# aerius-labs/paillier-halo2

Measured on AMD Instinct MI355X. Metric: Paillier-encrypt proofs/s (2048-bit n, k=17); MSM achieved HBM GB/s vs peak, higher is better.
Workload: dtype u32 limbs (29-bit reduced radix, 254-bit modular integers), u64 limbs (4096-bit integers)

## Files before the change

### paillier_halo2_amd/csrc/pz_msm.hip

```cpp
#include "ec.cuh"
#include "ec29.cuh"
#include "ec29_quad.cuh"
#include <math.h>
#include <stdlib.h>

#include "pz_internal.h"

#define MSM_CHUNK_MIN 16u
#define MSM_CHUNK_MAX 256u
#define MSM_HEAVY 24u
#define MSM_MEDIUM 1024u
#define MSM_SLICE_MAX_COLS 8u

struct MsmP {
    size_t n;
    size_t n_table;
    unsigned c;
    unsigned nwin;
    unsigned win_lo, win_hi;
    unsigned B;
    size_t cap;
    size_t max_items;
    unsigned chunk;
    unsigned spt;
// ... 132 lines not shown
            for (unsigned w = 0; w < p.win_hi; ++w) {
                int d = next_digit(s, w, p.c, carry);
                if (w >= p.win_lo && d != 0) atomicAdd(&h[(d < 0 ? -d : d) - 1], 1u);
            }
        }
    }
    __syncthreads();
    u32* out = slice_hist + (col * n_slices + slice) * (size_t)p.B;
    for (unsigned b = threadIdx.x; b < p.B; b += SORT_THREADS) out[b] = h[b];
}

__global__ __launch_bounds__(256) void k_msm_totals(u32* __restrict__ slice_hist, unsigned n_slices, MsmP p,
                                                    u32* __restrict__ totals) {
    const size_t col = blockIdx.y;
    const unsigned b = blockIdx.x * blockDim.x + threadIdx.x;
    if (b >= p.B) return;
    u32* sh = slice_hist + col * n_slices * (size_t)p.B + b;
    u32 run = 0;
    unsigned sl = 0;
    for (; sl + 8 <= n_slices; sl += 8) {
        u32 v[8];
#pragma unroll
        for (unsigned k = 0; k < 8; ++k) v[k] = sh[(size_t)(sl + k) * p.B];
#pragma unroll
        for (unsigned k = 0; k < 8; ++k) {
            sh[(size_t)(sl + k) * p.B] = run;
            run += v[k];
        }
    }
    for (; sl < n_slices; ++sl) {
        const u32 v = sh[(size_t)sl * p.B];
        sh[(size_t)sl * p.B] = run;
        run += v;
    }
    totals[col * p.B + b] = run;
}

#define ITEMS_SOLO 64u
#define SCAN_THREADS 1024
__global__ __launch_bounds__(SCAN_THREADS) void k_msm_scan(const u32* __restrict__ hist, MsmP p, u32* __restrict__ offs,
                                                  u32* __restrict__ items, u32* __restrict__ heavy,
                                                  u32* __restrict__ heavy_cnt, u32* __restrict__ fold_order,
                                                  u32* __restrict__ fold_cnt, u32* __restrict__ item_order,
                                                  u32* __restrict__ item_bucket, unsigned long long* __restrict__ digits_total) {
    __shared__ u32 s_cnt[SCAN_THREADS], s_itm[SCAN_THREADS];
    __shared__ u32 s_heavy;
    __shared__ u32 s_bin[MSM_HEAVY + 1], s_base[MSM_HEAVY + 1];
    __shared__ u32 s_obin[MSM_CHUNK_MAX + 1], s_obase[MSM_CHUNK_MAX + 1];
    if (threadIdx.x == 0) s_heavy = 0;
    if (threadIdx.x <= MSM_HEAVY) s_bin[threadIdx.x] = 0;
    for (unsigned t = threadIdx.x; t <= MSM_CHUNK_MAX; t += blockDim.x) s_obin[t] = 0;
    __syncthreads();
    const size_t col = blockIdx.x;
    const u32* h = hist + col * p.B;
    u32* o = offs + col * (p.B + 1);
    u32* it = items + col * (p.B + 1);
    const unsigned per = (p.B + SCAN_THREADS - 1) / SCAN_THREADS;
    const unsigned lo = threadIdx.x * per;
    u32 hv[32];
#pragma unroll
    for (unsigned k = 0; k < 32; ++k) hv[k] = (k < per && lo + k < p.B) ? h[lo + k] : 0u;
    u32 c = 0, m = 0;
#pragma unroll
    for (unsigned k = 0; k < 32; ++k) {
        const unsigned b = lo + k;
        if (k < per && b < p.B) {
// ... 62 lines not shown
            it[b] = m;
            c += v;
            const u32 ch = (v + p.chunk - 1) / p.chunk;
            m += ch;
            if (ch > 1 && ch <= MSM_HEAVY) fold_order[col * p.B + s_base[ch] + atomicAdd(&s_bin[ch], 1u)] = b;
            if (ch) {
                const u32 q = v / ch, rem = v % ch;
                const u32 ph = rem ? s_obase[q + 1] + atomicAdd(&s_obin[q + 1], rem) : 0u;
                const u32 pl = s_obase[q] + atomicAdd(&s_obin[q], ch - rem);
                {
                    const u32 item0 = m - ch;
                    u32* ord = item_order + col * p.max_items;
                    u32* obk = item_bucket + col * p.max_items;
                    for (u32 j = 0; j < ch; ++j) {
                        const u32 pos = j < rem ? ph + j : pl + j - rem;
                        ord[pos] = item0 + j;
                        obk[pos] = b;
                    }
                }
            }
        }
    }
}

#define SORT_FINE_LOG 7u
#define SORT_FINE (1u << SORT_FINE_LOG)
#define SORT_COARSE_MAX (SORT_MAXB >> SORT_FINE_LOG)
#define COARSE_THREADS 256u
#define COARSE_ROUND (COARSE_THREADS * 16u)
static_assert(COARSE_ROUND <= 65536u && SORT_COARSE_MAX <= 256u && SORT_COARSE_MAX == COARSE_THREADS, "k_msm_scatter_coarse packing");
__global__ __launch_bounds__(COARSE_THREADS) void k_msm_scatter_coarse(const Fr* __restrict__ scalars, size_t col_stride, MsmP p,
                                                                       const u32* __restrict__ slice_hist, unsigned n_slices,
                                                                       const u32* __restrict__ offs, u32* __restrict__ staged,
                                                                       size_t n_cols, ScatterSel sel) {
    if (!scatter_dense(sel)) return;
    __shared__ u32 cb[SORT_COARSE_MAX];
    __shared__ u32 cnt[SORT_COARSE_MAX];
    __shared__ u32 lbase[SORT_COARSE_MAX];
    __shared__ u32 gb[SORT_COARSE_MAX];
    __shared__ u32 stage[COARSE_ROUND];
    __shared__ unsigned char sbin[COARSE_ROUND];
    __shared__ u32 s_total;
    size_t col;
    unsigned slice;
    if (!sort_block_coords(n_slices, n_cols, slice, col)) return;
    const u32* in = slice_hist + (col * n_slices + slice) * (size_t)p.B;
    const u32* o = offs + col * (p.B + 1);
    const unsigned n_coarse = p.B >> SORT_FINE_LOG;
    if (threadIdx.x < SORT_COARSE_MAX) {
        cb[threadIdx.x] = threadIdx.x < n_coarse ? o[threadIdx.x << SORT_FINE_LOG] : 0u;
        cnt[threadIdx.x] = 0;
    }
    __syncthreads();
    for (unsigned b0 = (threadIdx.x & ~63u); b0 < p.B; b0 += 4 * COARSE_THREADS) {
        u32 v[4];
#pragma unroll
        for (unsigned k = 0; k < 4; ++k) {
            const unsigned b = b0 + k * COARSE_THREADS + (threadIdx.x & 63u);
            v[k] = b < p.B ? in[b] : 0u;
        }
#pragma unroll
        for (unsigned k = 0; k < 4; ++k) {
            u32 t = v[k];
#pragma unroll
            for (int off = 32; off > 0; off >>= 1) t += __shfl_xor(t, off, 64);
            const unsigned b = b0 + k * COARSE_THREADS;
            if ((threadIdx.x & 63u) == 0 && b < p.B && t) atomicAdd(&cb[b >> SORT_FINE_LOG], t);
        }
    }
    __syncthreads();
    u32* e = staged + col * p.cap;
    const size_t base = (size_t)slice * SORT_THREADS * p.spt;
    const unsigned rounds = SORT_THREADS * p.spt / COARSE_THREADS;
    Fr nxt = fp_zero<FrTag>();
    if (base + threadIdx.x < p.n) nxt = fp_load<FrTag>(scalars + col * col_stride + base + threadIdx.x);
    for (unsigned rd = 0; rd < rounds; ++rd) {
        const size_t i = base + (size_t)rd * COARSE_THREADS + threadIdx.x;
        if (base + (size_t)rd * COARSE_THREADS >= p.n) break;
        const Fr cur_scalar = nxt;
        u32 ev[16], rb[16];
#pragma unroll
        for (unsigned w = 0; w < 16; ++w) rb[w] = 0xffffffffu;
        if (i < p.n) {
            u32 s[8];
            const bool neg = scalar_prepare(cur_scalar, s);
            unsigned carry = 0;
#pragma unroll
// ... 719 lines not shown
    size_t i = (size_t)blockIdx.x * blockDim.x + threadIdx.x;
    if (i >= n) return;
    G1A29 a = x29_to_affine(x29_load_jac(in + i));
    if (!a29_is_inf(a)) {
        a.x = f29_to_256(a.x);
        a.y = f29_to_256(a.y);
    }
    a29_store64(out + i, a);
}

__global__ __launch_bounds__(128) void k_fixed_base_mul(const Fr* __restrict__ scalars, size_t n,
                                                        G1Aff64* __restrict__ out) {
    size_t i = (size_t)blockIdx.x * blockDim.x + threadIdx.x;
    if (i >= n) return;
    Fr k = fp_from_mont(fp_load<FrTag>(scalars + i));
    G1A29 g;
    g.x = f29_one<FqTag>();
    g.y = f29_canon<1>(f29_dbl(g.x));
    G1X29 acc = x29_inf();
    for (int bit = 253; bit >= 0; --bit) {
        acc = x29_dbl(acc);
        u32 w = sel8(k.v, (unsigned)bit >> 5);
        if ((w >> (bit & 31)) & 1) x29_add_affine(acc, g);
    }
    G1A29 a = x29_to_affine(acc);
    if (!a29_is_inf(a)) {
        a.x = f29_to_256(a.x);
        a.y = f29_to_256(a.y);
    }
    a29_store64(out + i, a);
}

static size_t pz_msm_ws_gib() {
    static size_t v = 0;
    if (!v) {
        const char* e = getenv("PZ_MSM_WS_GIB");
        long g = e ? atol(e) : 48;
        v = g < 1 ? 1 : (size_t)g;
    }
    return v;
}

static unsigned default_window_bits(size_t n) {
    if (n <= 1u << 8) return 9;
    if (n <= 1u << 11) return 11;
    if (n <= 1u << 14) return 13;
    return 16;
}

extern "C" int pz_bases_load_g1(pz_ctx* ctx, const uint64_t* bases_affine, size_t n_points, int on_device,
                                uint32_t window_bits, pz_bases** out) {
    if (!ctx || !out || !bases_affine || n_points == 0) return PZ_ERR_INVALID;
    *out = nullptr;
    unsigned c = window_bits ? window_bits : default_window_bits(n_points);
    if (c < 4 || c > 16) return PZ_ERR_INVALID;
    unsigned nwin = 253 / c + 1;
    if ((uint64_t)nwin * n_points >= (1ull << 31)) return PZ_ERR_UNSUPPORTED;
    PZ_ENTER(ctx);
    pz_bases* b = new pz_bases();
    b->n = n_points;
    b->c = c;
    b->nwin = nwin;
    b->device = ctx->device;
    hipError_t e = pz_hip_malloc(ctx, &b->d_table, (size_t)nwin * n_points * 64);
    if (e != hipSuccess) {
        delete b;
        return pz_hip_fail(ctx, e, "hipMalloc(table)");
    }
    const void* d_src = bases_affine;
    if (!on_device) {
        void* stage;
        int rc = pz_ws_get(ctx, WS_IO_A, n_points * 64, &stage);
        if (rc != PZ_OK) { (void)pz_hip_free(b->d_table); delete b; return rc; }
// ... 50 lines not shown
        unsigned c32 = ch < 24.0 ? MSM_CHUNK_MIN : 32u * (unsigned)((ch + 16.0) / 32.0);
        if (c32 > MSM_CHUNK_MAX) c32 = MSM_CHUNK_MAX;
        return c32;
    }
    const size_t want = (n_cols * digits_per_col) >> 18;
    unsigned chunk = MSM_CHUNK_MIN;
    while (chunk < MSM_CHUNK_MAX && chunk * 2 <= want) chunk *= 2;
    return chunk;
}

static unsigned msm_spt_for(size_t n_cols, size_t n) {
    const size_t min_wg = n_cols <= MSM_SLICE_MAX_COLS ? 128 : 512;
    unsigned spt = SORT_PER_THREAD;
    while (spt > 1 && n_cols * pz_div_up(n, (size_t)SORT_THREADS * spt) < min_wg) spt >>= 1;
    return spt;
}

#ifndef MSM_SPARSE_SLICE
#define MSM_SPARSE_SLICE (1u << 15)
#endif
static unsigned msm_spt_sparse(size_t n_cols, size_t n) {
    static long env = -1;
    if (env < 0) {
        const char* e = getenv("PZ_MSM_SPARSE_SLICE");
        env = e ? atol(e) : 0;
    }
    const size_t slice = env >= (long)SORT_SLICE && env <= (1l << 24) ? (size_t)env : (size_t)MSM_SPARSE_SLICE;
    unsigned spt = SORT_PER_THREAD;
    while ((size_t)SORT_THREADS * spt * 2 <= slice && (size_t)SORT_THREADS * spt < n) spt <<= 1;
    while (spt > 1 && n_cols * pz_div_up(n, (size_t)SORT_THREADS * spt) < 512) spt >>= 1;
    return spt;
}

static int msm_group(pz_ctx* ctx, const pz_bases* bases, const Fr* d_scalars, size_t nc, size_t n, size_t cs,
                     unsigned win_lo, unsigned win_hi, unsigned chunk, int density, G1Jac* d_out) {
    MsmP p;
    p.n = n;
    p.n_table = bases->n;
    p.c = bases->c;
    p.nwin = bases->nwin;
    p.win_lo = win_lo;
    p.win_hi = win_hi;
    p.B = 1u << (bases->c - 1);
    p.cap = n * (size_t)(win_hi - win_lo);
    p.chunk = chunk;
    if (p.B + n * (size_t)(win_hi - win_lo) / chunk > 65535u * 256u) return PZ_ERR_CAPACITY;
    p.max_items = p.B + p.cap / chunk;
    void *hist, *offs, *heavy, *items, *entries, *partials, *na, *nb, *totals, *fold, *iord;
    static int scatter_mode = -1;
    if (scatter_mode < 0) {
        const char* e = getenv("PZ_MSM_SCATTER");
        scatter_mode = (e && !strcmp(e, "one")) ? 1 : (e && !strcmp(e, "two")) ? 2 : 0;
    }
    const bool batch = nc > MSM_SLICE_MAX_COLS;
    const bool hint_sparse = batch && scatter_mode == 0 && density == PZ_MSM_SPARSE;
    const bool hint_dense = batch && scatter_mode == 0 && density == PZ_MSM_DENSE;
    p.spt = hint_sparse ? msm_spt_sparse(nc, n) : msm_spt_for(nc, n);
    const unsigned n_slices = pz_div_up(n, (size_t)SORT_THREADS * p.spt);
    const bool one_slice = hint_sparse && n_slices == 1;
    PZCHK(pz_ws_get(ctx, WS_HIST, nc * (size_t)n_slices * p.B * 4, &hist));
    PZCHK(pz_ws_get(ctx, WS_CURSOR, nc * (size_t)(p.B + 1) * 4, &heavy));
    const bool split_items = nc <= MSM_SLICE_MAX_COLS;
    const unsigned nblk_few = pz_div_up(p.B, 256);
    PZCHK(pz_ws_get(ctx, WS_TOTALS, nc * ((size_t)p.B + (split_items ? (size_t)nblk_few * (2 + FEW_BINS) : 0)) * 4, &totals));
    u32* blk_cnt = (u32*)totals + nc * (size_t)p.B;
    u32* blk_itm = blk_cnt + nc * (size_t)nblk_few;
    u32* blk_bins = blk_itm + nc * (size_t)nblk_few;
    u32* heavy_cnt = (u32*)heavy + nc * (size_t)p.B;
    PZCHK(pz_ws_get(ctx, WS_MISC, nc * (size_t)(p.B + 1) * 4, &fold));
    u32* fold_cnt = (u32*)fold + nc * (size_t)p.B;
    PZCHK(pz_ws_get(ctx, WS_ORDER, nc * p.max_items * 8, &iord));
    u32* item_order = (u32*)iord;
    u32* item_bucket = (u32*)iord + nc * p.max_items;
    PZCHK(pz_ws_get(ctx, WS_OFFS, nc * (p.B + 1) * 4, &offs));
    PZCHK(pz_ws_get(ctx, WS_ITEMS, nc * (p.B + 1) * 4, &items));
    PZCHK(pz_ws_get(ctx, WS_ENTRIES, nc * p.cap * 4 + 16, &entries));
    const bool two_pass = scatter_mode != 1 && !hint_sparse && p.c == 16 && (size_t)p.nwin * p.n_table <= ((size_t)1 << 24) &&
                          (nc > MSM_SLICE_MAX_COLS || scatter_mode == 2);
    {
        const size_t part_bytes = nc * p.max_items * sizeof(G1X29Raw), stage_bytes = two_pass ? nc * p.cap * 4 + 16 : 0;
        PZCHK(pz_ws_get(ctx, WS_PARTIALS, part_bytes > stage_bytes ? part_bytes : stage_bytes, &partials));
    }
    const unsigned m1 = p.B >= 16 ? 16 : p.B;
    unsigned n_nodes = p.B / m1;
    PZCHK(pz_ws_get(ctx, WS_NODES_A, nc * (size_t)n_nodes * sizeof(MsmNode), &na));
    PZCHK(pz_ws_get(ctx, WS_NODES_B, nc * (size_t)(n_nodes / 2 + 1) * sizeof(MsmNode), &nb));
    hipStream_t st = ctx->stream;
    pz_timer tall(ctx, PZ_T_MSM_ALL);
    dim3 gs(sort_grid(n_slices, nc));
    void* dsel;
    PZCHK(pz_ws_get(ctx, WS_SEL, 8, &dsel));
    HIPCHK(ctx, hipMemsetAsync(dsel, 0, 8, st));
    PZCHK(pz_async_err_init(ctx));
    {
        pz_timer tsort(ctx, PZ_T_MSM_SORT);
        hipLaunchKernelGGL(k_msm_hist, gs, dim3(SORT_THREADS), 0, st, d_scalars, cs, p, (u32*)hist, n_slices, nc);
        if (split_items) {
            hipLaunchKernelGGL(k_msm_totals_few, dim3(nblk_few, (unsigned)nc), dim3(256), 0, st, (u32*)hist, n_slices, p, (u32*)totals,
                               blk_cnt, blk_itm, blk_bins);
            hipLaunchKernelGGL(k_msm_items_few, dim3(nblk_few, (unsigned)nc), dim3(256), 0, st, p, (const u32*)totals, (const u32*)blk_cnt,
                               (const u32*)blk_itm, (const u32*)blk_bins, (u32*)offs, (u32*)items, item_order, item_bucket,
                               (unsigned long long*)dsel);
        } else {
            if (!one_slice)
                hipLaunchKernelGGL(k_msm_totals, dim3(pz_div_up(p.B, 256), (unsigned)nc), dim3(256), 0, st, (u32*)hist, n_slices, p,
                                   (u32*)totals);
            hipLaunchKernelGGL(k_msm_scan, dim3((unsigned)nc), dim3(SCAN_THREADS), 0, st, (const u32*)(one_slice ? hist : totals), p,
                               (u32*)offs, (u32*)items, (u32*)heavy, heavy_cnt, (u32*)fold, fold_cnt, item_order, item_bucket,
                               (unsigned long long*)dsel);
        }
        ScatterSel sel;
        sel.total = (const unsigned long long*)dsel;
        sel.thr = !two_pass ? ~0ull : (scatter_mode == 2 || hint_dense) ? 0ull : (unsigned long long)(0.4 * (double)nc * (double)p.cap);
        sel.err = ctx->async_err_d;
        if (two_pass) {
            hipLaunchKernelGGL(k_msm_scatter_coarse, gs, dim3(COARSE_THREADS), 0, st, d_scalars, cs, p, (const u32*)hist, n_slices,
                               (const u32*)offs, (u32*)partials, nc, sel);
            hipLaunchKernelGGL(k_msm_scatter_fine, dim3(p.B >> SORT_FINE_LOG, (unsigned)nc), dim3(FINE_THREADS), 0, st, p, (const u32*)offs,
                               (const u32*)partials, (u32*)entries, sel);
        }
        if (!two_pass || (scatter_mode != 2 && !hint_dense))
            hipLaunchKernelGGL(k_msm_scatter, gs, dim3(SORT_THREADS), 0, st, d_scalars, cs, p, one_slice ? (const u32*)nullptr : (const u32*)hist,
                               n_slices, (const u32*)offs, (u32*)entries, nc, sel);
    }
    {
        pz_timer tacc(ctx, PZ_T_MSM_ACC);
        hipLaunchKernelGGL(k_msm_accumulate, dim3((unsigned)nc, pz_div_up(p.max_items, 256)), dim3(256), 0, st,
                           (const G1Aff64*)bases->d_table, p, (const u32*)offs, (const u32*)items,
                           (const u32*)item_order, (const u32*)item_bucket, (const u32*)entries, (G1X29Raw*)partials);
    }
    pz_timer ttree(ctx, PZ_T_MSM_TREE);
    if (split_items) {
        const unsigned gx4 = pz_div_up(p.B, 64), gx32 = p.B / 8 < 2048u ? (p.B / 8 ? p.B / 8 : 1u) : 2048u;
        hipLaunchKernelGGL(k_msm_fold_few, dim3(gx4, (unsigned)nc), dim3(256), 0, st, p, (const u32*)items, (G1X29Raw*)partials, 2u, 1u, MSM_FEW_SMALL);
        hipLaunchKernelGGL(k_msm_fold_few, dim3(gx32, (unsigned)nc), dim3(256), 0, st, p, (const u32*)items, (G1X29Raw*)partials, 5u, MSM_FEW_SMALL,
                           MSM_MEDIUM);
        hipLaunchKernelGGL(k_msm_heavy_few, dim3(p.B / 256 < 64u ? (p.B / 256 ? p.B / 256 : 1u) : 64u, (unsigned)nc), dim3(256), 0, st, p,
                           (const u32*)items, (G1X29Raw*)partials);
    } else {
    hipLaunchKernelGGL(k_msm_bucket_sum, dim3((unsigned)nc, pz_div_up(p.B, 256)), dim3(256), 0, st, p, (const u32*)items,
                       (const u32*)fold, (const u32*)fold_cnt, (G1X29Raw*)partials);
    unsigned hx = (unsigned)(8192 / nc);
    if (hx < 4) hx = 4;
    if (hx > p.B) hx = p.B;
    hipLaunchKernelGGL(k_msm_heavy_sum, dim3(hx, (unsigned)nc), dim3(256), 0, st, p, (const u32*)items, (const u32*)heavy,
                       (const u32*)heavy_cnt, (G1X29Raw*)partials);
    hipLaunchKernelGGL(k_msm_medium_sum, dim3(hx, (unsigned)nc), dim3(256), 0, st, p, (const u32*)items, (const u32*)heavy,
                       (const u32*)heavy_cnt, (G1X29Raw*)partials);
    }
    if (nc <= MSM_SLICE_MAX_COLS) {
// ... 49 lines not shown
        PZCHK(pz_ws_get(ctx, WS_NODES_A, nn * sizeof(MsmNode), &z));
        HIPCHK(ctx, hipMemsetAsync(z, 0, nn * sizeof(MsmNode), ctx->stream));
        hipLaunchKernelGGL(k_msm_emit, dim3(pz_div_up(nn, 64)), dim3(64), 0, ctx->stream, (const MsmNode*)z, nn,
                           (G1Jac*)d_out_jac);
        HIPCHK(ctx, hipGetLastError());
        return PZ_OK;
    }
    const size_t cs = col_stride / 4;
    const size_t digits = n * (size_t)(win_hi - win_lo);
    const unsigned chunk = msm_chunk_for(n_cols, digits, bases->c);
    const size_t part_col = (digits / chunk) * sizeof(G1X29Raw);
    size_t per_col = digits * 4 + (part_col > digits * 4 ? part_col : digits * 4) + (digits / chunk) * 8 +
                     (size_t)(1u << (bases->c - 1)) * (180 + 4 * (size_t)pz_div_up(n, (size_t)SORT_THREADS * msm_spt_for(1, n)));
    size_t ws_budget = pz_msm_ws_gib() << 30;
    {
        if (ctx->mem_avail == 0 || ++ctx->mem_avail_age >= 64) {
            const size_t free_b = pz_mem_free_bytes(ctx);
            if (free_b) {
                size_t held = 0;
                for (int i = 0; i < WS_COUNT; ++i) held += ctx->ws[i].cap;
                ctx->mem_avail = (free_b + held) / 2;
                ctx->mem_avail_age = 0;
            }
        }
        if (ctx->mem_avail && ws_budget > ctx->mem_avail) ws_budget = ctx->mem_avail;
    }
    size_t group = ws_budget / per_col;
    if (group == 0) group = 1;
    if (group > n_cols) group = n_cols;
    if (group > 4096) group = 4096;
    if (density == PZ_MSM_SPARSE && group > MSM_SLICE_MAX_COLS) {
        const size_t slices = pz_div_up(n, (size_t)SORT_THREADS * msm_spt_sparse(group, n));
        per_col = digits * 4 + part_col + (digits / chunk) * 8 + (size_t)(1u << (bases->c - 1)) * (180 + 4 * slices);
        group = ws_budget / per_col;
        if (group > n_cols) group = n_cols;
        if (group > 4096) group = 4096;
    }
    for (size_t c0 = 0; c0 < n_cols;) {
        const size_t nc = n_cols - c0 < group ? n_cols - c0 : group;
        const int rc = msm_group(ctx, bases, (const Fr*)d_scalars + c0 * cs, nc, n, cs, win_lo, win_hi, chunk, density, (G1Jac*)d_out_jac + c0);
        if (rc == PZ_ERR_OOM && group > 1) {
            ctx->mem_avail = 0;
            (void)hipGetLastError();
            group = (group + 1) / 2;
            continue;
        }
        PZCHK(rc);
        c0 += nc;
    }
    return PZ_OK;
}

extern "C" int pz_msm_g1_batch(pz_ctx* ctx, const pz_bases* bases, const uint64_t* const* scalar_cols, size_t n_cols,
                               size_t n, uint64_t* out_jac) {
    if (!ctx || !bases || (n_cols && (!scalar_cols || !out_jac))) return PZ_ERR_INVALID;
    if (n > bases->n) return PZ_ERR_INVALID;
    if (n_cols == 0) return PZ_OK;
    PZ_ENTER(ctx);
    const size_t bytes = n * 32;
    for (size_t j = 0; j < n_cols; ++j)
        if (!scalar_cols[j] && n) return PZ_ERR_INVALID;
    const size_t g_min = bytes ? (((size_t)1 << 27) / bytes ? ((size_t)1 << 27) / bytes : 1) : n_cols;
    size_t g_max = bytes ? (((size_t)1 << 30) / bytes ? ((size_t)1 << 30) / bytes : 1) : n_cols;
    if (g_max > n_cols) g_max = n_cols;
    void *d_s, *d_o;
    PZCHK(pz_ws_get(ctx, WS_IO_B, 2 * g_max * bytes + 32, &d_s));
// ... 258 lines not shown
```

### paillier_halo2_amd/csrc/pz_quotient.hip

```cpp
#include "fp29.cuh"
#include "pz_internal.h"

static inline Fr fp_one_host() {
    static const uint64_t ONE[4] = {0xac96341c4ffffffbULL, 0x36fc76959f60cd29ULL, 0x666ea36f7879462eULL, 0x0e0a77c19a07df2fULL};
    Fr r;
    memcpy(r.v, ONE, 32);
    return r;
}
static inline Fr fr_from_u64(const uint64_t x[4]) {
    Fr r;
    memcpy(r.v, x, 32);
    return r;
}

typedef F29<FrTag> Fr29;
__device__ __forceinline__ Fr29 fr29_c261(const Fr& c) { return f29_to_261(f29_from_fp(c)); }
__device__ __forceinline__ Fr29 fr29_one256() {
    Fr29 r;
#pragma unroll
    for (int i = 0; i < 9; ++i) r.v[i] = P29<FrTag>::R256(i);
    return r;
}

struct S29 {
// ... 196 lines not shown
        if (threadIdx.x >= off) {
#pragma unroll
            for (int i = 0; i < 9; ++i) u.v[i] = s[i * 256 + threadIdx.x - off];
        }
        __syncthreads();
        if (threadIdx.x >= off) {
            p = f29_mul(u, p);
#pragma unroll
            for (int i = 0; i < 9; ++i) s[i * 256 + threadIdx.x] = p.v[i];
        }
        __syncthreads();
    }
    Fr29 e = f29_one<FrTag>();
    if (threadIdx.x) {
#pragma unroll
        for (int i = 0; i < 9; ++i) e.v[i] = s[i * 256 + threadIdx.x - 1];
    }
    Fr w;
    f29_pack(e, w.v);
    fp_store(excl + (size_t)blockIdx.y * nb * 256 + t, w);
    if (threadIdx.x == 255) f29_store_product(block_tot + (size_t)blockIdx.y * nb + blockIdx.x, f29_to_256(p));
}
__global__ void k_pp_blocks(Fr* __restrict__ block_tot, unsigned nb, size_t n_cols, Fr z0) {
    const size_t col = (size_t)blockIdx.x * blockDim.x + threadIdx.x;
    if (col >= n_cols) return;
    Fr* bt = block_tot + col * nb;
    Fr run = z0;
    for (unsigned b = 0; b < nb; ++b) {
        Fr t = fp_load<FrTag>(bt + b);
        fp_store(bt + b, run);
        run = fp_mul(run, t);
    }
}
__global__ __launch_bounds__(256) void k_pp_apply(const Fr* __restrict__ a, size_t as, size_t n, const Fr* __restrict__ excl,
                                                  const Fr* __restrict__ block_tot, unsigned nb, Fr* __restrict__ z, size_t zs) {
    a += (size_t)blockIdx.y * as;
    z += (size_t)blockIdx.y * zs;
    const size_t t = (size_t)blockIdx.x * 256 + threadIdx.x;
    const size_t lo = t * PP_K;
    if (lo >= n) return;
    Fr29 cur = f29_mul(f29_load<FrTag>(block_tot + (size_t)blockIdx.y * nb + blockIdx.x),
                       f29_load<FrTag>(excl + (size_t)blockIdx.y * nb * 256 + t));
    for (unsigned j = 0; j < PP_K && lo + j < n; ++j) {
        const Fr v = fp_load<FrTag>(a + lo + j);
        f29_store_product(z + lo + j, cur);
        cur = f29_mul(cur, f29_from_fp_shl5(v));
    }
}

int pz_prefix_product_batch_internal(pz_ctx* ctx, const Fr* d_a, size_t a_stride, size_t n_cols, size_t n, Fr z0, Fr* d_z,
                                     size_t z_stride) {
    if (!n || !n_cols) return PZ_OK;
    if (n_cols > 65535) return PZ_ERR_INVALID;
    const unsigned nb = pz_div_up(pz_div_up(n, PP_K), 256);
    void* ws;
    PZCHK(pz_ws_get(ctx, WS_BIG_B, n_cols * ((size_t)nb * 256 + nb) * 32, &ws));
    Fr* excl = (Fr*)ws;
    Fr* tot = excl + n_cols * (size_t)nb * 256;
    hipLaunchKernelGGL(k_pp_local, dim3(nb, (unsigned)n_cols), dim3(256), 0, ctx->stream, d_a, a_stride, n, excl, tot, nb);
    hipLaunchKernelGGL(k_pp_blocks, dim3(pz_div_up(n_cols, 64)), dim3(64), 0, ctx->stream, tot, nb, n_cols, z0);
    hipLaunchKernelGGL(k_pp_apply, dim3(nb, (unsigned)n_cols), dim3(256), 0, ctx->stream, d_a, a_stride, n, (const Fr*)excl,
                       (const Fr*)tot, nb, d_z, z_stride);
    HIPCHK(ctx, hipGetLastError());
    return PZ_OK;
}
int pz_prefix_product_internal(pz_ctx* ctx, const Fr* d_a, size_t n, Fr z0, Fr* d_z) {
    return pz_prefix_product_batch_internal(ctx, d_a, n, 1, n, z0, d_z, n);
}

extern "C" int pz_fr_prefix_product_dev(pz_ctx* ctx, const uint64_t* d_a, size_t n, const uint64_t z0[4], uint64_t* d_z) {
    if (!ctx || !z0 || (n && (!d_a || !d_z))) return PZ_ERR_INVALID;
    PZ_ENTER(ctx);
    return pz_prefix_product_internal(ctx, (const Fr*)d_a, n, fr_from_u64(z0), (Fr*)d_z);
}

__global__ __launch_bounds__(256) void k_perm_terms(const Fr* __restrict__ cols, size_t cs, const Fr* __restrict__ sigma,
                                                    size_t ss, unsigned m, size_t n, const Fr* __restrict__ wpow, Fr beta,
                                                    Fr gamma, Fr delta0, Fr delta, Fr* __restrict__ num,
                                                    Fr* __restrict__ den) {
    const size_t i = (size_t)blockIdx.x * blockDim.x + threadIdx.x;
    if (i >= n) return;
    const Fr29 g = fr29_c261(gamma), d = fr29_c261(delta), beta266 = f29_to_261(fr29_c261(beta));
    Fr29 nm = fr29_one256(), dn = nm;
    Fr29 bd = f29_mul(f29_mul(beta266, f29_from_fp(delta0)), f29_load_shl5<FrTag>(wpow + i));
    for (unsigned j = 0; j < m; ++j) {
        const Fr29 v = f29_add(f29_load_shl5<FrTag>(cols + (size_t)j * cs + i), g);
        const Fr29 sg = f29_load<FrTag>(sigma + (size_t)j * ss + i);
        nm = f29_mul(nm, f29_add(v, bd));
        dn = f29_mul(dn, f29_add(v, f29_mul(beta266, sg)));
        bd = f29_mul(bd, d);
    }
    f29_store<0>(num + i, nm);
    f29_store<0>(den + i, dn);
}

// ... 14 lines not shown
    Fr* den = num + n;
    hipLaunchKernelGGL(k_perm_terms, dim3(pz_div_up(n, 256)), dim3(256), 0, ctx->stream, (const Fr*)d_cols, col_stride / 4,
                       (const Fr*)d_sigma, sigma_stride / 4, (unsigned)m, n, (const Fr*)wp, fr_from_u64(beta), fr_from_u64(gamma),
                       fr_from_u64(delta_start), fr_from_u64(delta), num, den);
    HIPCHK(ctx, hipGetLastError());
    PZCHK(pz_batch_invert_internal(ctx, den, n, num));
    return pz_prefix_product_internal(ctx, num, n, fr_from_u64(z0), (Fr*)d_z);
}

__global__ __launch_bounds__(256) void k_perm_terms_sets(const Fr* __restrict__ cols, size_t cs, const Fr* __restrict__ sigma,
                                                         size_t ss, unsigned m, unsigned chunk_len, size_t n,
                                                         const Fr* __restrict__ wpow, const Fr* __restrict__ dpow,
                                                         S29 beta266, S29 g, S29 d, Fr* __restrict__ num, Fr* __restrict__ den,
                                                         unsigned set0) {
    const size_t i = (size_t)blockIdx.x * blockDim.x + threadIdx.x;
    if (i >= n) return;
    const unsigned c0 = (set0 + blockIdx.y) * chunk_len, set = blockIdx.y;
    Fr29 nm = fr29_one256(), dn = nm;
    Fr29 bd = f29_mul(f29_mul_s(f29_load<FrTag>(dpow + c0), beta266.v), f29_load_shl5<FrTag>(wpow + i));
    Fr v_n = fp_load<FrTag>(cols + (size_t)c0 * cs + i), s_n = fp_load<FrTag>(sigma + (size_t)c0 * ss + i);
    for (unsigned c = c0; c < c0 + chunk_len && c < m; ++c) {
        const Fr29 v = f29_add_s(f29_from_fp_shl5(v_n), g.v);
        const Fr29 sg = f29_from_fp(s_n);
        const unsigned cn = (c + 1 < c0 + chunk_len && c + 1 < m) ? c + 1 : c;
        v_n = fp_load<FrTag>(cols + (size_t)cn * cs + i);
        s_n = fp_load<FrTag>(sigma + (size_t)cn * ss + i);
        nm = f29_mul(nm, f29_add(v, bd));
        dn = f29_mul(dn, f29_add(v, f29_mul_s(sg, beta266.v)));
        bd = f29_mul_s(bd, d.v);
    }
    f29_store_product(num + (size_t)set * n + i, nm);
    f29_store_product(den + (size_t)set * n + i, dn);
}
__global__ __launch_bounds__(256) void k_perm_chain(const Fr* __restrict__ z, size_t zs, unsigned n_sets, size_t u, Fr* __restrict__ mult) {
    __shared__ Fr s_p[256];
    const unsigned per = (n_sets + 255u) / 256u, lo = threadIdx.x * per, hi = lo + per < n_sets ? lo + per : n_sets;
    Fr p = fp_one<FrTag>();
    for (unsigned j = lo; j < hi; ++j) p = fp_mul(p, fp_load<FrTag>(z + (size_t)j * zs + u));
    s_p[threadIdx.x] = p;
    __syncthreads();
    for (unsigned off = 1; off < 256; off <<= 1) {
        Fr v = fp_one<FrTag>();
        if (threadIdx.x >= off) v = s_p[threadIdx.x - off];
        __syncthreads();
        if (threadIdx.x >= off) {
            p = fp_mul(v, p);
            s_p[threadIdx.x] = p;
        }
        __syncthreads();
    }
    Fr c = threadIdx.x ? s_p[threadIdx.x - 1] : fp_one<FrTag>();
    for (unsigned j = lo; j < hi; ++j) {
        fp_store(mult + j, c);
        c = fp_mul(c, fp_load<FrTag>(z + (size_t)j * zs + u));
    }
}
__global__ __launch_bounds__(256) void k_scale_sets(Fr* __restrict__ z, size_t zs, size_t n, const Fr* __restrict__ mult) {
    const size_t i = (size_t)blockIdx.x * blockDim.x + threadIdx.x;
    if (i >= n || blockIdx.y == 0) return;
    Fr* p = z + (size_t)blockIdx.y * zs + i;
    fp_store(p, fp_mul(fp_load<FrTag>(p), fp_load<FrTag>(mult + blockIdx.y)));
}

extern "C" int pz_permutation_product_sets_dev(pz_ctx* ctx, const uint64_t* d_cols, size_t col_stride, const uint64_t* d_sigma,
                                               size_t sigma_stride, size_t m, uint32_t chunk_len, uint32_t log_n,
                                               size_t usable_rows, const uint64_t omega[4], const uint64_t beta[4],
                                               const uint64_t gamma[4], const uint64_t delta[4], uint64_t* d_z,
                                               size_t z_stride) {
    if (!ctx || !d_cols || !d_sigma || !d_z || !omega || !beta || !gamma || !delta || m == 0 || chunk_len == 0 || log_n > 26)
        return PZ_ERR_INVALID;
    const size_t n = (size_t)1 << log_n;
    const size_t n_sets = (m + chunk_len - 1) / chunk_len;
    if (col_stride % 4 || sigma_stride % 4 || z_stride % 4 || usable_rows >= n || n_sets > 65535 || m > 0xffffffu) return PZ_ERR_INVALID;
    if ((m > 1 && (col_stride < 4 * n || sigma_stride < 4 * n)) || (n_sets > 1 && z_stride < 4 * n)) return PZ_ERR_INVALID;
    if (!host_fr_canonical(beta) || !host_fr_canonical(gamma) || !host_fr_canonical(delta)) return PZ_ERR_INVALID;
    PZ_ENTER(ctx);
    void *wp, *dp, *ws, *mu;
    PZCHK(pz_get_pow_table(ctx, omega, n, &wp));
    PZCHK(pz_get_pow_table(ctx, delta, m, &dp));
    size_t sb = ((size_t)4 << 30) / (2 * n * 32);
    if (sb < 1) sb = 1;
    if (sb > n_sets) sb = n_sets;
    PZCHK(pz_ws_get(ctx, WS_BIG_C, 2 * sb * n * 32, &ws));
    PZCHK(pz_ws_get(ctx, WS_MISC, n_sets * 32, &mu));
    Fr* num = (Fr*)ws;
    Fr* den = num + sb * n;
    for (size_t s0 = 0; s0 < n_sets; s0 += sb) {
        const size_t ns = n_sets - s0 < sb ? n_sets - s0 : sb;
        hipLaunchKernelGGL(k_perm_terms_sets, dim3(pz_div_up(n, 256), (unsigned)ns), dim3(256), 0, ctx->stream,
                           (const Fr*)d_cols, col_stride / 4, (const Fr*)d_sigma, sigma_stride / 4, (unsigned)m, (unsigned)chunk_len, n,
                           (const Fr*)wp, (const Fr*)dp, host_fr_shl(beta, 10), host_fr_shl(gamma, 5), host_fr_shl(delta, 5), num, den,
                           (unsigned)s0);
        HIPCHK(ctx, hipGetLastError());
        PZCHK(pz_batch_invert_internal(ctx, den, ns * n, num));
        PZCHK(pz_prefix_product_batch_internal(ctx, num, n, ns, n, fp_one_host(), (Fr*)d_z + s0 * (z_stride / 4), z_stride / 4));
    }
    if (n_sets > 1) {
        hipLaunchKernelGGL(k_perm_chain, dim3(1), dim3(256), 0, ctx->stream, (const Fr*)d_z, z_stride / 4, (unsigned)n_sets,
                           usable_rows, (Fr*)mu);
        hipLaunchKernelGGL(k_scale_sets, dim3(pz_div_up(n, 256), (unsigned)n_sets), dim3(256), 0, ctx->stream, (Fr*)d_z,
                           z_stride / 4, n, (const Fr*)mu);
        HIPCHK(ctx, hipGetLastError());
    }
    return PZ_OK;
}

__global__ __launch_bounds__(256) void k_quotient_gate(const Fr* __restrict__ adv, size_t as, const Fr* __restrict__ sel,
                                                       size_t ss, unsigned n_cols, size_t N, unsigned step, S29 y261,
                                                       Fr* __restrict__ h) {
    const size_t i = (size_t)blockIdx.x * blockDim.x + threadIdx.x;
    if (i >= N) return;
    const size_t i1 = (i + step) & (N - 1), i2 = (i + 2 * (size_t)step) & (N - 1), i3 = (i + 3 * (size_t)step) & (N - 1);
    Fr29 acc = f29_load<FrTag>(h + i);
    for (unsigned j = 0; j < n_cols; ++j) {
        const Fr* a = adv + (size_t)j * as;
        const Fr29 a0 = f29_load<FrTag>(a + i), a1 = f29_load<FrTag>(a + i1), a3 = f29_load<FrTag>(a + i3);
        const Fr29 a2 = f29_load_shl5<FrTag>(a + i2), sl = f29_load_shl5<FrTag>(sel + (size_t)j * ss + i);
        const Fr29 e = f29_sub<2, 29>(f29_add(a0, f29_mul(a1, a2)), a3);
        acc = f29_mul2_s(acc, y261.v, e, sl);
    }
    f29_store<0>(h + i, acc);
}

extern "C" int pz_quotient_gate_dev(pz_ctx* ctx, const uint64_t* d_adv_ext, size_t adv_stride, const uint64_t* d_sel_ext,
                                    size_t sel_stride, size_t n_cols, uint32_t log_ext, uint32_t rot_step,
                                    const uint64_t y[4], uint64_t* d_h) {
    if (!ctx || !y || !d_h || log_ext > 28 || (n_cols && (!d_adv_ext || !d_sel_ext))) return PZ_ERR_INVALID;
    if (adv_stride % 4 || sel_stride % 4 || n_cols > 0xffffffffu) return PZ_ERR_INVALID;
    const size_t N = (size_t)1 << log_ext;
    if (rot_step == 0 || rot_step >= N) return PZ_ERR_INVALID;
    if (n_cols > 1 && (adv_stride < 4 * N || sel_stride < 4 * N)) return PZ_ERR_INVALID;
    if (!host_fr_canonical(y)) return PZ_ERR_INVALID;
    if (n_cols == 0) return PZ_OK;
    PZ_ENTER(ctx);
    hipLaunchKernelGGL(k_quotient_gate, dim3(pz_div_up(N, 256)), dim3(256), 0, ctx->stream, (const Fr*)d_adv_ext,
// ... 534 lines not shown
```

Before: 1.444.

## Precompute per-slice coarse offsets for dense MSM sort; fold permutation chaining into prefix product

```diff
diff --git a/paillier_halo2_amd/csrc/pz_msm.hip b/paillier_halo2_amd/csrc/pz_msm.hip
--- a/paillier_halo2_amd/csrc/pz_msm.hip
+++ b/paillier_halo2_amd/csrc/pz_msm.hip
@@ -188,6 +188,41 @@
         const u32 v = sh[(size_t)sl * p.B];
         sh[(size_t)sl * p.B] = run;
         run += v;
+    }
+    totals[col * p.B + b] = run;
+}
+
+#define TOTALS_GROUP_SLICES 32u
+static_assert(TOTALS_GROUP_SLICES * 2u <= 256u, "k_msm_totals_groups: one thread per (slice, group) of a step");
+__global__ __launch_bounds__(256) void k_msm_totals_groups(const u32* __restrict__ slice_hist, unsigned n_slices, MsmP p,
+                                                           u32* __restrict__ totals, u32* __restrict__ group_offs) {
+    __shared__ u32 s_w[TOTALS_GROUP_SLICES * 4];
+    const size_t col = blockIdx.y;
+    const unsigned b = blockIdx.x * 256 + threadIdx.x;
+    const unsigned n_coarse = p.B >> 7, lane = threadIdx.x & 63u, wv = threadIdx.x >> 6;
+    const u32* sh = slice_hist + col * n_slices * (size_t)p.B + b;
+    u32 run = 0;
+    for (unsigned s0 = 0; s0 < n_slices; s0 += TOTALS_GROUP_SLICES) {
+        const unsigned ns = n_slices - s0 < TOTALS_GROUP_SLICES ? n_slices - s0 : TOTALS_GROUP_SLICES;
+        for (unsigned k0 = 0; k0 < ns; k0 += 8) {
+            u32 v[8];
+#pragma unroll
+            for (unsigned k = 0; k < 8; ++k) v[k] = k0 + k < ns ? sh[(size_t)(s0 + k0 + k) * p.B] : 0u;
+#pragma unroll
+            for (unsigned k = 0; k < 8; ++k) {
+                u32 t = run;
+#pragma unroll
+                for (int off = 32; off > 0; off >>= 1) t += __shfl_xor(t, off, 64);
+                if (lane == 0 && k0 + k < ns) s_w[(k0 + k) * 4 + wv] = t;
+                run += v[k];
+            }
+        }
+        __syncthreads();
+        if (threadIdx.x < ns * 2) {
+            const unsigned sl = threadIdx.x >> 1, h = threadIdx.x & 1u;
+            group_offs[(col * n_slices + s0 + sl) * n_coarse + blockIdx.x * 2 + h] = s_w[sl * 4 + 2 * h] + s_w[sl * 4 + 2 * h + 1];
+        }
+        __syncthreads();
     }
     totals[col * p.B + b] = run;
 }
@@ -316,7 +351,7 @@
 __global__ __launch_bounds__(COARSE_THREADS) void k_msm_scatter_coarse(const Fr* __restrict__ scalars, size_t col_stride, MsmP p,
                                                                        const u32* __restrict__ slice_hist, unsigned n_slices,
                                                                        const u32* __restrict__ offs, u32* __restrict__ staged,
-                                                                       size_t n_cols, ScatterSel sel) {
+                                                                       size_t n_cols, ScatterSel sel, const u32* __restrict__ group_offs) {
     if (!scatter_dense(sel)) return;
     __shared__ u32 cb[SORT_COARSE_MAX];
     __shared__ u32 cnt[SORT_COARSE_MAX];
@@ -328,15 +363,17 @@
     size_t col;
     unsigned slice;
     if (!sort_block_coords(n_slices, n_cols, slice, col)) return;
-    const u32* in = slice_hist + (col * n_slices + slice) * (size_t)p.B;
+    const u32* in = slice_hist ? slice_hist + (col * n_slices + slice) * (size_t)p.B : nullptr;
     const u32* o = offs + col * (p.B + 1);
     const unsigned n_coarse = p.B >> SORT_FINE_LOG;
     if (threadIdx.x < SORT_COARSE_MAX) {
-        cb[threadIdx.x] = threadIdx.x < n_coarse ? o[threadIdx.x << SORT_FINE_LOG] : 0u;
+        u32 c0 = threadIdx.x < n_coarse ? o[threadIdx.x << SORT_FINE_LOG] : 0u;
+        if (group_offs && threadIdx.x < n_coarse) c0 += group_offs[(col * n_slices + slice) * n_coarse + threadIdx.x];
+        cb[threadIdx.x] = c0;
         cnt[threadIdx.x] = 0;
     }
     __syncthreads();
-    for (unsigned b0 = (threadIdx.x & ~63u); b0 < p.B; b0 += 4 * COARSE_THREADS) {
+    for (unsigned b0 = (threadIdx.x & ~63u); slice_hist && b0 < p.B; b0 += 4 * COARSE_THREADS) {
         u32 v[4];
 #pragma unroll
         for (unsigned k = 0; k < 4; ++k) {
@@ -1122,13 +1159,9 @@
 }
 
 static size_t pz_msm_ws_gib() {
-    static size_t v = 0;
-    if (!v) {
-        const char* e = getenv("PZ_MSM_WS_GIB");
-        long g = e ? atol(e) : 48;
-        v = g < 1 ? 1 : (size_t)g;
-    }
-    return v;
+    const char* e = getenv("PZ_MSM_WS_GIB");
+    const long g = e ? atol(e) : 48;
+    return g < 1 ? 1 : (size_t)g;
 }
 
 static unsigned default_window_bits(size_t n) {
@@ -1245,6 +1278,33 @@
     return spt;
 }
 
+#ifndef MSM_DENSE_SLICE
+#define MSM_DENSE_SLICE (1u << 15)
+#endif
+static unsigned msm_spt_dense(size_t n_cols, size_t n) {
+    const char* e = getenv("PZ_MSM_DENSE_SLICE");
+    const long env = e ? atol(e) : 0;
+    const size_t slice = env >= (long)SORT_SLICE && env <= (1l << 24) ? (size_t)env : (size_t)MSM_DENSE_SLICE;
+    unsigned spt = SORT_PER_THREAD;
+    while ((size_t)SORT_THREADS * spt * 2 <= slice && (size_t)SORT_THREADS * spt < n) spt <<= 1;
+    while (spt > 1 && n_cols * pz_div_up(n, (size_t)SORT_THREADS * spt) < 512) spt >>= 1;
+    return spt;
+}
+
+static int msm_scatter_mode() {
+    static int mode = -1;
+    if (mode < 0) {
+        const char* e = getenv("PZ_MSM_SCATTER");
+        mode = (e && !strcmp(e, "one")) ? 1 : (e && !strcmp(e, "two")) ? 2 : 0;
+    }
+    return mode;
+}
+
+static bool msm_dense_two_step(const pz_bases* bases, size_t nc, int density) {
+    return nc > MSM_SLICE_MAX_COLS && msm_scatter_mode() == 0 && density == PZ_MSM_DENSE && bases->c == 16 &&
+           (size_t)bases->nwin * bases->n <= ((size_t)1 << 24);
+}
+
 static int msm_group(pz_ctx* ctx, const pz_bases* bases, const Fr* d_scalars, size_t nc, size_t n, size_t cs,
                      unsigned win_lo, unsigned win_hi, unsigned chunk, int density, G1Jac* d_out) {
     MsmP p;
@@ -1260,18 +1320,17 @@
     if (p.B + n * (size_t)(win_hi - win_lo) / chunk > 65535u * 256u) return PZ_ERR_CAPACITY;
     p.max_items = p.B + p.cap / chunk;
     void *hist, *offs, *heavy, *items, *entries, *partials, *na, *nb, *totals, *fold, *iord;
-    static int scatter_mode = -1;
-    if (scatter_mode < 0) {
-        const char* e = getenv("PZ_MSM_SCATTER");
-        scatter_mode = (e && !strcmp(e, "one")) ? 1 : (e && !strcmp(e, "two")) ? 2 : 0;
-    }
+    const int scatter_mode = msm_scatter_mode();
     const bool batch = nc > MSM_SLICE_MAX_COLS;
     const bool hint_sparse = batch && scatter_mode == 0 && density == PZ_MSM_SPARSE;
     const bool hint_dense = batch && scatter_mode == 0 && density == PZ_MSM_DENSE;
-    p.spt = hint_sparse ? msm_spt_sparse(nc, n) : msm_spt_for(nc, n);
+    const bool dense_lean = msm_dense_two_step(bases, nc, density);
+    p.spt = hint_sparse ? msm_spt_sparse(nc, n) : dense_lean ? msm_spt_dense(nc, n) : msm_spt_for(nc, n);
     const unsigned n_slices = pz_div_up(n, (size_t)SORT_THREADS * p.spt);
-    const bool one_slice = hint_sparse && n_slices == 1;
-    PZCHK(pz_ws_get(ctx, WS_HIST, nc * (size_t)n_slices * p.B * 4, &hist));
+    const bool one_slice = (hint_sparse || dense_lean) && n_slices == 1;
+    const unsigned n_coarse = p.B >> SORT_FINE_LOG;
+    PZCHK(pz_ws_get(ctx, WS_HIST, nc * (size_t)n_slices * ((size_t)p.B + (dense_lean ? n_coarse : 0u)) * 4, &hist));
+    u32* group_offs = (u32*)hist + nc * (size_t)n_slices * p.B;
     PZCHK(pz_ws_get(ctx, WS_CURSOR, nc * (size_t)(p.B + 1) * 4, &heavy));
     const bool split_items = nc <= MSM_SLICE_MAX_COLS;
     const unsigned nblk_few = pz_div_up(p.B, 256);
@@ -1315,9 +1374,13 @@
                                (const u32*)blk_itm, (const u32*)blk_bins, (u32*)offs, (u32*)items, item_order, item_bucket,
                                (unsigned long long*)dsel);
         } else {
-            if (!one_slice)
+            if (!one_slice && dense_lean) {
+                hipLaunchKernelGGL(k_msm_totals_groups, dim3(p.B / 256, (unsigned)nc), dim3(256), 0, st, (const u32*)hist, n_slices, p,
+                                   (u32*)totals, group_offs);
+            } else if (!one_slice) {
                 hipLaunchKernelGGL(k_msm_totals, dim3(pz_div_up(p.B, 256), (unsigned)nc), dim3(256), 0, st, (u32*)hist, n_slices, p,
                                    (u32*)totals);
+            }
             hipLaunchKernelGGL(k_msm_scan, dim3((unsigned)nc), dim3(SCAN_THREADS), 0, st, (const u32*)(one_slice ? hist : totals), p,
                                (u32*)offs, (u32*)items, (u32*)heavy, heavy_cnt, (u32*)fold, fold_cnt, item_order, item_bucket,
                                (unsigned long long*)dsel);
@@ -1327,8 +1390,9 @@
         sel.thr = !two_pass ? ~0ull : (scatter_mode == 2 || hint_dense) ? 0ull : (unsigned long long)(0.4 * (double)nc * (double)p.cap);
         sel.err = ctx->async_err_d;
         if (two_pass) {
-            hipLaunchKernelGGL(k_msm_scatter_coarse, gs, dim3(COARSE_THREADS), 0, st, d_scalars, cs, p, (const u32*)hist, n_slices,
-                               (const u32*)offs, (u32*)partials, nc, sel);
+            hipLaunchKernelGGL(k_msm_scatter_coarse, gs, dim3(COARSE_THREADS), 0, st, d_scalars, cs, p,
+                               dense_lean ? (const u32*)nullptr : (const u32*)hist, n_slices, (const u32*)offs, (u32*)partials, nc, sel,
+                               dense_lean && !one_slice ? (const u32*)group_offs : (const u32*)nullptr);
             hipLaunchKernelGGL(k_msm_scatter_fine, dim3(p.B >> SORT_FINE_LOG, (unsigned)nc), dim3(FINE_THREADS), 0, st, p, (const u32*)offs,
                                (const u32*)partials, (u32*)entries, sel);
         }
@@ -1444,6 +1508,15 @@
     if (density == PZ_MSM_SPARSE && group > MSM_SLICE_MAX_COLS) {
         const size_t slices = pz_div_up(n, (size_t)SORT_THREADS * msm_spt_sparse(group, n));
         per_col = digits * 4 + part_col + (digits / chunk) * 8 + (size_t)(1u << (bases->c - 1)) * (180 + 4 * slices);
+        group = ws_budget / per_col;
+        if (group > n_cols) group = n_cols;
+        if (group > 4096) group = 4096;
+    } else if (density == PZ_MSM_DENSE && group > MSM_SLICE_MAX_COLS) {
+        const bool lean = msm_dense_two_step(bases, group, density);
+        const size_t slices = pz_div_up(n, (size_t)SORT_THREADS * (lean ? msm_spt_dense(group, n) : msm_spt_for(group, n)));
+        const size_t B = (size_t)1 << (bases->c - 1);
+        per_col = digits * 4 + (part_col > digits * 4 ? part_col : digits * 4) + (digits / chunk) * 8 + B * (180 + 4 * slices) +
+                  (lean ? (B >> SORT_FINE_LOG) * 4 * slices : 0);
         group = ws_budget / per_col;
         if (group > n_cols) group = n_cols;
         if (group > 4096) group = 4096;
diff --git a/paillier_halo2_amd/csrc/pz_quotient.hip b/paillier_halo2_amd/csrc/pz_quotient.hip
--- a/paillier_halo2_amd/csrc/pz_quotient.hip
+++ b/paillier_halo2_amd/csrc/pz_quotient.hip
@@ -252,8 +252,18 @@
         run = fp_mul(run, t);
     }
 }
+__global__ void k_pp_row_value(const Fr* __restrict__ a, size_t as, size_t n_cols, size_t u, const Fr* __restrict__ excl,
+                               const Fr* __restrict__ block_tot, unsigned nb, Fr* __restrict__ zu) {
+    const size_t col = (size_t)blockIdx.x * blockDim.x + threadIdx.x;
+    if (col >= n_cols) return;
+    const size_t t = u / PP_K, lo = t * PP_K;
+    Fr29 cur = f29_mul(f29_load<FrTag>(block_tot + col * nb + t / 256), f29_load<FrTag>(excl + col * nb * 256 + t));
+    for (size_t i = lo; i < u; ++i) cur = f29_mul(cur, f29_load_shl5<FrTag>(a + col * as + i));
+    f29_store_product(zu + col, cur);
+}
 __global__ __launch_bounds__(256) void k_pp_apply(const Fr* __restrict__ a, size_t as, size_t n, const Fr* __restrict__ excl,
-                                                  const Fr* __restrict__ block_tot, unsigned nb, Fr* __restrict__ z, size_t zs) {
+                                                  const Fr* __restrict__ block_tot, unsigned nb, Fr* __restrict__ z, size_t zs,
+                                                  const Fr* __restrict__ mult) {
     a += (size_t)blockIdx.y * as;
     z += (size_t)blockIdx.y * zs;
     const size_t t = (size_t)blockIdx.x * 256 + threadIdx.x;
@@ -261,6 +271,7 @@
     if (lo >= n) return;
     Fr29 cur = f29_mul(f29_load<FrTag>(block_tot + (size_t)blockIdx.y * nb + blockIdx.x),
                        f29_load<FrTag>(excl + (size_t)blockIdx.y * nb * 256 + t));
+    if (mult) cur = f29_mul(cur, f29_load_shl5<FrTag>(mult + blockIdx.y));
     for (unsigned j = 0; j < PP_K && lo + j < n; ++j) {
         const Fr v = fp_load<FrTag>(a + lo + j);
         f29_store_product(z + lo + j, cur);
@@ -268,8 +279,47 @@
     }
 }
 
+struct PpChain {
+    size_t u;
+    Fr* zu;
+    Fr* mult;
+    Fr* carry;
+    bool first;
+};
+__global__ __launch_bounds__(256) void k_perm_chain(const Fr* __restrict__ z, size_t zs, unsigned n_sets, size_t u, Fr* __restrict__ mult,
+                                                    Fr* __restrict__ carry, int first) {
+    __shared__ Fr s_p[256];
+    const unsigned per = (n_sets + 255u) / 256u, lo = threadIdx.x * per, hi = lo + per < n_sets ? lo + per : n_sets;
+    const Fr c0 = first ? fp_one<FrTag>() : fp_load<FrTag>(carry);
+    Fr p = fp_one<FrTag>();
+    for (unsigned j = lo; j < hi; ++j) p = fp_mul(p, fp_load<FrTag>(z + (size_t)j * zs + u));
+    s_p[threadIdx.x] = p;
+    __syncthreads();
+    for (unsigned off = 1; off < 256; off <<= 1) {
+        Fr v = fp_one<FrTag>();
+        if (threadIdx.x >= off) v = s_p[threadIdx.x - off];
+        __syncthreads();
+        if (threadIdx.x >= off) {
+            p = fp_mul(v, p);
+            s_p[threadIdx.x] = p;
+        }
+        __syncthreads();
+    }
+    if (threadIdx.x == 255) fp_store(carry, fp_mul(c0, p));
+    Fr c = threadIdx.x ? fp_mul(c0, s_p[threadIdx.x - 1]) : c0;
+    for (unsigned j = lo; j < hi; ++j) {
+        fp_store(mult + j, c);
+        c = fp_mul(c, fp_load<FrTag>(z + (size_t)j * zs + u));
+    }
+}
+static int pp_batch(pz_ctx* ctx, const Fr* d_a, size_t a_stride, size_t n_cols, size_t n, Fr z0, Fr* d_z, size_t z_stride,
+                    const PpChain* chain);
 int pz_prefix_product_batch_internal(pz_ctx* ctx, const Fr* d_a, size_t a_stride, size_t n_cols, size_t n, Fr z0, Fr* d_z,
                                      size_t z_stride) {
+    return pp_batch(ctx, d_a, a_stride, n_cols, n, z0, d_z, z_stride, nullptr);
+}
+static int pp_batch(pz_ctx* ctx, const Fr* d_a, size_t a_stride, size_t n_cols, size_t n, Fr z0, Fr* d_z, size_t z_stride,
+                    const PpChain* chain) {
     if (!n || !n_cols) return PZ_OK;
     if (n_cols > 65535) return PZ_ERR_INVALID;
     const unsigned nb = pz_div_up(pz_div_up(n, PP_K), 256);
@@ -279,8 +329,14 @@
     Fr* tot = excl + n_cols * (size_t)nb * 256;
     hipLaunchKernelGGL(k_pp_local, dim3(nb, (unsigned)n_cols), dim3(256), 0, ctx->stream, d_a, a_stride, n, excl, tot, nb);
     hipLaunchKernelGGL(k_pp_blocks, dim3(pz_div_up(n_cols, 64)), dim3(64), 0, ctx->stream, tot, nb, n_cols, z0);
+    if (chain) {
+        hipLaunchKernelGGL(k_pp_row_value, dim3(pz_div_up(n_cols, 64)), dim3(64), 0, ctx->stream, d_a, a_stride, n_cols, chain->u,
+                           (const Fr*)excl, (const Fr*)tot, nb, chain->zu);
+        hipLaunchKernelGGL(k_perm_chain, dim3(1), dim3(256), 0, ctx->stream, (const Fr*)chain->zu, (size_t)1, (unsigned)n_cols, (size_t)0,
+                           chain->mult, chain->carry, chain->first ? 1 : 0);
+    }
     hipLaunchKernelGGL(k_pp_apply, dim3(nb, (unsigned)n_cols), dim3(256), 0, ctx->stream, d_a, a_stride, n, (const Fr*)excl,
-                       (const Fr*)tot, nb, d_z, z_stride);
+                       (const Fr*)tot, nb, d_z, z_stride, chain ? (const Fr*)chain->mult : (const Fr*)nullptr);
     HIPCHK(ctx, hipGetLastError());
     return PZ_OK;
 }
@@ -361,35 +417,6 @@
     f29_store_product(num + (size_t)set * n + i, nm);
     f29_store_product(den + (size_t)set * n + i, dn);
 }
-__global__ __launch_bounds__(256) void k_perm_chain(const Fr* __restrict__ z, size_t zs, unsigned n_sets, size_t u, Fr* __restrict__ mult) {
-    __shared__ Fr s_p[256];
-    const unsigned per = (n_sets + 255u) / 256u, lo = threadIdx.x * per, hi = lo + per < n_sets ? lo + per : n_sets;
-    Fr p = fp_one<FrTag>();
-    for (unsigned j = lo; j < hi; ++j) p = fp_mul(p, fp_load<FrTag>(z + (size_t)j * zs + u));
-    s_p[threadIdx.x] = p;
-    __syncthreads();
-    for (unsigned off = 1; off < 256; off <<= 1) {
-        Fr v = fp_one<FrTag>();
-        if (threadIdx.x >= off) v = s_p[threadIdx.x - off];
-        __syncthreads();
-        if (threadIdx.x >= off) {
-            p = fp_mul(v, p);
-            s_p[threadIdx.x] = p;
-        }
-        __syncthreads();
-    }
-    Fr c = threadIdx.x ? s_p[threadIdx.x - 1] : fp_one<FrTag>();
-    for (unsigned j = lo; j < hi; ++j) {
-        fp_store(mult + j, c);
-        c = fp_mul(c, fp_load<FrTag>(z + (size_t)j * zs + u));
-    }
-}
-__global__ __launch_bounds__(256) void k_scale_sets(Fr* __restrict__ z, size_t zs, size_t n, const Fr* __restrict__ mult) {
-    const size_t i = (size_t)blockIdx.x * blockDim.x + threadIdx.x;
-    if (i >= n || blockIdx.y == 0) return;
-    Fr* p = z + (size_t)blockIdx.y * zs + i;
-    fp_store(p, fp_mul(fp_load<FrTag>(p), fp_load<FrTag>(mult + blockIdx.y)));
-}
 
 extern "C" int pz_permutation_product_sets_dev(pz_ctx* ctx, const uint64_t* d_cols, size_t col_stride, const uint64_t* d_sigma,
                                                size_t sigma_stride, size_t m, uint32_t chunk_len, uint32_t log_n,
@@ -408,10 +435,15 @@
     PZCHK(pz_get_pow_table(ctx, omega, n, &wp));
     PZCHK(pz_get_pow_table(ctx, delta, m, &dp));
     size_t sb = ((size_t)4 << 30) / (2 * n * 32);
+    if (const char* e = getenv("PZ_PERM_SET_BATCH")) {
+        const long v = atol(e);
+        if (v >= 1 && (size_t)v < sb) sb = (size_t)v;
+    }
     if (sb < 1) sb = 1;
     if (sb > n_sets) sb = n_sets;
     PZCHK(pz_ws_get(ctx, WS_BIG_C, 2 * sb * n * 32, &ws));
-    PZCHK(pz_ws_get(ctx, WS_MISC, n_sets * 32, &mu));
+    PZCHK(pz_ws_get(ctx, WS_MISC, (2 * sb + 1) * 32, &mu));
+    PpChain chain = {usable_rows, (Fr*)mu, (Fr*)mu + sb, (Fr*)mu + 2 * sb, true};
     Fr* num = (Fr*)ws;
     Fr* den = num + sb * n;
     for (size_t s0 = 0; s0 < n_sets; s0 += sb) {
@@ -422,14 +454,8 @@
                            (unsigned)s0);
         HIPCHK(ctx, hipGetLastError());
         PZCHK(pz_batch_invert_internal(ctx, den, ns * n, num));
-        PZCHK(pz_prefix_product_batch_internal(ctx, num, n, ns, n, fp_one_host(), (Fr*)d_z + s0 * (z_stride / 4), z_stride / 4));
-    }
-    if (n_sets > 1) {
-        hipLaunchKernelGGL(k_perm_chain, dim3(1), dim3(256), 0, ctx->stream, (const Fr*)d_z, z_stride / 4, (unsigned)n_sets,
-                           usable_rows, (Fr*)mu);
-        hipLaunchKernelGGL(k_scale_sets, dim3(pz_div_up(n, 256), (unsigned)n_sets), dim3(256), 0, ctx->stream, (Fr*)d_z,
-                           z_stride / 4, n, (const Fr*)mu);
-        HIPCHK(ctx, hipGetLastError());
+        chain.first = s0 == 0;
+        PZCHK(pp_batch(ctx, num, n, ns, n, fp_one_host(), (Fr*)d_z + s0 * (z_stride / 4), z_stride / 4, n_sets > 1 ? &chain : nullptr));
     }
     return PZ_OK;
 }
diff --git a/profiles/probes/dense_sort_slices.py b/profiles/probes/dense_sort_slices.py
--- /dev/null
+++ b/profiles/probes/dense_sort_slices.py
@@ -0,0 +1,48 @@
+import os, sys, time
+sys.path.insert(0, os.path.dirname(os.path.dirname(os.path.dirname(os.path.abspath(__file__)))))
+import numpy as np
+import torch
+import paillier_halo2_amd as pz
+
+nc, n = int(os.environ.get("COLS", "768")), 1 << int(os.environ.get("LOG_N", "17"))
+reps = int(os.environ.get("REPS", "5"))
+eng = pz.Engine(0)
+eng.bind_torch_stream()
+s, t = (0x2B7 << 236) + 0x4321, 0xFEEDC0DE1234567
+ks = np.frombuffer(b"".join(int(s + i * t).to_bytes(32, "little") for i in range(n)), dtype="<u8").reshape(-1, 4).copy()
+d_k = torch.from_numpy(ks.view(np.int64)).cuda()
+eng.fr_convert_dev(d_k.data_ptr(), n, True)
+d_b = torch.zeros((n, 8), dtype=torch.int64, device="cuda")
+eng.g1_fixed_base_mul_dev(d_k.data_ptr(), n, d_b.data_ptr())
+eng.sync()
+tb = eng.load_bases_dev(d_b.data_ptr(), n, window_bits=16)
+gen = torch.Generator(device="cuda")
+gen.manual_seed(0x5043)
+d_s = torch.randint(-(1 << 63), (1 << 63) - 1, (nc, n, 4), dtype=torch.int64, device="cuda", generator=gen)
+d_s[:, :, 3] &= 0x0FFFFFFFFFFFFFFF
+eng.fr_convert_dev(d_s.data_ptr(), nc * n, True)
+d_o = torch.zeros((nc, 12), dtype=torch.int64, device="cuda")
+eng.timing_enable(True)
+outs = {}
+modes = os.environ.get("MODES", "auto,8192,16384,32768,%d,default,auto,32768,8192" % n).split(",")
+for name in modes:
+    hint = None if name == "auto" else pz.MSM_DENSE
+    os.environ.pop("PZ_MSM_DENSE_SLICE", None)
+    if name not in ("auto", "default"):
+        os.environ["PZ_MSM_DENSE_SLICE"] = name
+    fn = lambda: eng.msm_dev(tb, d_s.data_ptr(), nc, n, 4 * n, d_o.data_ptr(), density=hint)
+    fn(); eng.sync()
+    outs[name] = d_o.cpu().numpy().copy()
+    eng.timing_reset()
+    t0 = time.perf_counter()
+    for _ in range(reps):
+        fn()
+    eng.sync()
+    dt = (time.perf_counter() - t0) / reps
+    sort, acc, tree, whole = (eng.timing_get(w)[0] / reps for w in (5, 0, 6, 4))
+    print("slice=%-7s cols=%d  sort %.2f ms  accumulate %.2f ms  tree %.2f ms  msm %.2f ms  wall %.2f ms" % (
+        name, nc, sort, acc, tree, whole, dt * 1e3), flush=True)
+if len(outs) > 1:
+    pts = {k: eng.g1_normalize(v.view(np.uint64)) for k, v in outs.items()}
+    first = next(iter(pts.values()))
+    print("same points:", all(bool(np.array_equal(first, p)) for p in pts.values()), flush=True)
```

New measurement: 1.456 (median of 6 runs). No clear change (+0.8%).
